# osudrl/cassie-mujoco-sim

Measured on AMD Instinct MI355X. Metric: env-steps/sec (whole node) at N envs; max |qpos_err| vs CPU ref, higher is better.
Workload: dtype f64

## Files before the change

### cassie-mujoco-sim_amd/csrc/env_step_rows.inc

```
        int r_ = lane;
        int rtype = -1, rid = 0, rsub = 0;
        int nefc = 0, nefc_before_contacts = 0;
        double rpos = 0, rmargin = 0, rR = 1.0, rK = 0, rB = 0, rimp = 1.0;
        const bool need_imu = lastsub || io.all_outputs_every_substep || (io.drive_mode && sub + 2 == nsub);
        const bool need_pos = lastsub || io.drive_mode || io.all_outputs_every_substep;
        const bool issens = lane < m->nsensor && need_pos;
        const int ls = issens ? lane : 0;
        SensorConsts sens_c;
        double ycol[NVP];
        double jvel = 0, jws = 0;
        const bool lastcol = !WIDE && lane == NROW - 1;
        for (int pass = 0; pass < (WIDE ? 2 : 1); ++pass) {
        if constexpr (WIDE) {
            if (pass == 1 && nefc <= NROW) break;
            r_ = NROW * pass + lane; rtype = -1; rid = 0; rsub = 0; nefc = 0; jvel = 0; jws = 0;
            rpos = 0; rmargin = 0; rR = 1.0; rK = 0; rB = 0; rimp = 1.0;
        }
        {
            const int neq = m->neq;
            const bool eact = lane < neq && m->eq_active[lane < neq ? lane : 0] != 0;
            const unsigned long long eall = neq >= 64 ? ~0ull : (1ull << neq) - 1;
            if (wv::ballot(eact) == eall && 3 * neq <= capr) {
                if (r_ < 3 * neq) { rtype = CM_CNSTR_EQUALITY; rid = r_ / 3; rsub = r_ - 3 * rid; }
                nefc = 3 * neq;
            } else
            for (int e = 0; e < neq; ++e) {
                if (!m->eq_active[e]) continue;
                if (nefc + 3 > capr) { warn |= WARN_CONSTRAINT_FULL; continue; }
                if (r_ >= nefc && r_ < nefc + 3) { rtype = CM_CNSTR_EQUALITY; rid = e; rsub = r_ - nefc; }
                nefc += 3;
            }
        }
        {
            for (unsigned long long any = lob | hib; any; any &= any - 1) {
                const int j = wv::popc64((any & (0ull - any)) - 1);
                for (int side = 0; side < 2; ++side) {
                    if (!(((side == 0 ? lob : hib) >> j) & 1ull)) continue;
                    if (nefc >= capr) { warn |= WARN_CONSTRAINT_FULL; continue; }
                    if (r_ == nefc) { rtype = CM_CNSTR_LIMIT_JOINT; rid = j; rsub = side; }
                    ++nefc;
                }
            }
        }
        nefc_before_contacts = nefc;
        const bool cpyr = lane < ncon && S.c_dim[lane < ncon ? lane : 0] == 3;
        if (wv::ballot(cpyr) == (ncon >= 64 ? ~0ull : (1ull << ncon) - 1) && nefc + 4 * ncon <= capr) {
            if (r_ >= nefc && r_ < nefc + 4 * ncon) { rtype = CM_CNSTR_CONTACT_PYRAMIDAL; rid = (r_ - nefc) >> 2; rsub = (r_ - nefc) & 3; }
            nefc += 4 * ncon;
        } else
        for (int c = 0; c < ncon; ++c) {
            const int dim = S.c_dim[c];
            if (dim != 1 && dim != 3) { warn |= WARN_UNSUPPORTED_PAIR; continue; }
            const int nrow = dim == 1 ? 1 : 2 * (dim - 1);
            if (nefc + nrow > capr) { warn |= WARN_CONSTRAINT_FULL; continue; }
            if (r_ >= nefc && r_ < nefc + nrow) {
                rtype = dim == 1 ? CM_CNSTR_CONTACT_FRICTIONLESS : CM_CNSTR_CONTACT_PYRAMIDAL;
                rid = c; rsub = r_ - nefc;
            }
            nefc += nrow;
        }

        CK_STAMP(25);
        double u3[3] = {0, 0, 0}, wp[3] = {0, 0, 0}, wm[3] = {0, 0, 0};
        unsigned long long maskp = 0, maskm = 0;
        int limdof = -1;
        double limsgn = 0, rdiag = 0, imp_pos = 0, rRscale = 1.0;
        double solref0 = 0.02, solref1 = 1, solimp[5] = {0.9, 0.95, 0.001, 0.5, 2};
        if (rtype == CM_CNSTR_EQUALITY) {
            if (rid != pf_eq) {
                pf_eb1 = m->eq_body1[rid]; pf_eb2 = m->eq_body2[rid]; pf_er1 = m->eq_root[rid][0]; pf_er2 = m->eq_root[rid][1];
            }
            maskp = m->eq_dofmask[rid][0]; maskm = m->eq_dofmask[rid][1];
            rdiag = P->eq_invweight[rid];
            solref0 = m->eq_solref[rid][0]; solref1 = m->eq_solref[rid][1];
            for (int i = 0; i < 5; ++i) solimp[i] = m->eq_solimp[rid][i];
            const int b1 = pf_eb1, b2 = pf_eb2;
            double l1[3] = {m->eq_data[rid][0], m->eq_data[rid][1], m->eq_data[rid][2]};
            double l2[3] = {m->eq_data[rid][3], m->eq_data[rid][4], m->eq_data[rid][5]};
            double a1[3], a2[3];
            mulmatvec3(a1, S.x.s.xmat[b1], l1);
            mulmatvec3(a2, S.x.s.xmat[b2], l2);
            for (int i = 0; i < 3; ++i) { a1[i] += S.x.s.xpos[b1][i]; a2[i] += S.x.s.xpos[b2][i]; }
            u3[0] = rsub == 0 ? 1.0 : 0.0; u3[1] = rsub == 1 ? 1.0 : 0.0; u3[2] = rsub == 2 ? 1.0 : 0.0;
            const double *c1 = S.com[pf_er1], *c2 = S.com[pf_er2];
            double o1[3] = {a1[0] - c1[0], a1[1] - c1[1], a1[2] - c1[2]};
            double o2[3] = {a2[0] - c2[0], a2[1] - c2[1], a2[2] - c2[2]};
            cross3(wp, o1, u3);
            cross3(wm, o2, u3);

            double res[3] = {a1[0] - a2[0], a1[1] - a2[1], a1[2] - a2[2]};
            rpos = rsub == 0 ? res[0] : (rsub == 1 ? res[1] : res[2]); rmargin = 0;
            imp_pos = sqrt(dot3(res, res));

        } else if (rtype == CM_CNSTR_LIMIT_JOINT) {
            const double q = S.qpos[m->jnt_qposadr[rid]];
            rpos = rsub == 0 ? q - m->jnt_range[rid][0] : m->jnt_range[rid][1] - q;
            rmargin = m->jnt_margin[rid];
            imp_pos = rpos;
            limdof = m->jnt_dofadr[rid];
            limsgn = rsub == 0 ? 1.0 : -1.0;
            rdiag = P->jnt_liminvweight[rid];
            solref0 = m->jnt_solref[rid][0]; solref1 = m->jnt_solref[rid][1];
            for (int i = 0; i < 5; ++i) solimp[i] = m->jnt_solimp[rid][i];
        } else if (rtype >= 0) {
            const int c = rid;
            const double *fr = S.c_frame[c];
            if (rtype == CM_CNSTR_CONTACT_PYRAMIDAL) {
                const int a = 1 + rsub / 2;
                const double mu = a <= 2 ? S.c_fri[c][0] : (a == 3 ? S.c_fri[c][1] : S.c_fri[c][2]);
                const double sg = (rsub & 1) ? -mu : mu;
                for (int i = 0; i < 3; ++i) u3[i] = fr[i] + sg * fr[3 * a + i];
                const double mu0 = S.c_fri[c][0];
                rRscale = 2 * mu0 * mu0;
            } else {
                for (int i = 0; i < 3; ++i) u3[i] = fr[i];
            }
            const double *c1 = S.com[S.c_root[c][0]], *c2 = S.com[S.c_root[c][1]];
            double o1[3] = {S.c_pos[c][0] - c1[0], S.c_pos[c][1] - c1[1], S.c_pos[c][2] - c1[2]};
            double o2[3] = {S.c_pos[c][0] - c2[0], S.c_pos[c][1] - c2[1], S.c_pos[c][2] - c2[2]};
            cross3(wp, o2, u3);
            cross3(wm, o1, u3);
            maskp = S.c_dofmask[c][1];
            maskm = S.c_dofmask[c][0];
            rpos = S.c_dist[c]; rmargin = S.c_margin[c]; imp_pos = rpos;
            const double tran = S.c_tran[c];
            const double mu_first = S.c_fri[c][0];
            rdiag = rtype == CM_CNSTR_CONTACT_PYRAMIDAL ? tran + mu_first * mu_first * tran : tran;
            solref0 = S.c_solref[c][0]; solref1 = S.c_solref[c][1];
            for (int i = 0; i < 5; ++i) solimp[i] = S.c_solimp[c][i];
        }
        CK_STAMP(26);
        if (rtype >= 0) {
            rimp = impedance(solimp, imp_pos, rmargin);
            rR = fmax(CM_MINVAL, (1 - rimp) * rdiag / rimp);
            if (rtype == CM_CNSTR_CONTACT_PYRAMIDAL) rR = fmax(CM_MINVAL, rRscale * rR);
            const double dmax = solimp[1];
            if (solref0 > 0) {
                double tc = solref0;
                if ((m->flags & CM_FLAG_REFSAFE) && tc < 2 * h) tc = 2 * h;
                rK = 1.0 / fmax(CM_MINVAL, dmax * dmax * tc * tc * solref1 * solref1);
                rB = 2.0 / fmax(CM_MINVAL, dmax * tc);
            } else {
                rK = -solref0 / fmax(CM_MINVAL, dmax * dmax);
                rB = -solref1 / fmax(CM_MINVAL, dmax);
            }
        }
        CK_STAMP(27);
        if constexpr (NW == 1) sens_c = request_sensor_consts(m, ls);
#pragma unroll
        for (int k0 = 0; k0 < NVP; k0 += 4) {
            double cc[4][6], qv[4], qw[4], qs[4];
#pragma unroll
            for (int kk = 0; kk < 4; ++kk) {
#pragma unroll
                for (int t = 0; t < 6; ++t) cc[kk][t] = S.cdof[k0 + kk][t];
                qv[kk] = S.qvel[k0 + kk]; qw[kk] = S.qacc_ws[k0 + kk];
                if constexpr (NW == 1) qs[kk] = S.qfrc_smooth[k0 + kk]; else qs[kk] = 0.0;
            }
            wv::sched_fence();
#pragma unroll
            for (int kk = 0; kk < 4; ++kk) {
                const int k = k0 + kk;
                double v = 0;
                if (TOPO::is_static ? k < TOPO::nv : k < nv) {
                    if (rtype >= 0) {
                        const double ul = u3[0] * cc[kk][3] + u3[1] * cc[kk][4] + u3[2] * cc[kk][5];
                        const double sp = bitf(maskp, k), sm = bitf(maskm, k);
                        v = sp * (ul + wp[0] * cc[kk][0] + wp[1] * cc[kk][1] + wp[2] * cc[kk][2]) -
                            sm * (ul + wm[0] * cc[kk][0] + wm[1] * cc[kk][1] + wm[2] * cc[kk][2]);
                        if (k == limdof) v = limsgn;
                        jvel += v * qv[kk];
                        jws += v * qw[kk];
                    } else if (lastcol) {
                        v = qs[kk];
                    }
                }
                ycol[k] = v;
            }
        }
        if constexpr (WIDE) {
            if (r_ < MAXR) {
#pragma unroll
                for (int k = 0; k < NVP; ++k) S.x.Yr[r_][k] = ycol[k];
                double *rt = S.x.rowt[r_];
                rt[0] = rR; rt[1] = rtype >= 0 ? -rB * jvel - rK * rimp * (rpos - rmargin) : 0.0; rt[2] = jws;
                rt[3] = rtype < 0 ? -1.0 : (rtype == CM_CNSTR_EQUALITY ? 0.0 : 1.0);
            }
            if (readout_ext<FEAT>(io) && pass == 0 && rtype == CM_CNSTR_EQUALITY && r_ < CM_MAXEQROW) {
                cm_ext_t *ex = readout_ext<FEAT>(io) + env;
                ex->eq_pos[r_] = rpos; ex->eq_id[r_] = rid;
#pragma unroll
                for (int k = 0; k < NVP; ++k) if (k < nv) ex->eq_J[r_][k] = ycol[k];
            }
        }
        }
        const int sb = NW == 1 ? sens_c.sb : 0;
        CK_STAMP(28);
        if constexpr (NW == 2) {
            if constexpr (WIDE) { if (lane == 0) S.x.turn[0] = nefc; }
            CK_STAMP(34); wv::block_barrier();
            if (lastcol) {
#pragma unroll
                for (int k = 0; k < NVP; ++k) ycol[k] = (TOPO::is_static ? k < TOPO::nv : k < nv) ? S.qfrc_smooth[k] : 0.0;
            }
        }
        const double raref = rtype >= 0 ? -rB * jvel - rK * rimp * (rpos - rmargin) : 0.0;

        int aslot = -1;
        if constexpr (NW == 1) aslot = sensors_before_solve(io, S, m, env, issens, ls, sens_c, need_imu, lastsub);
        CK_STAMP(29);
        if (io.xpos_out && isbody && lastsub) {
            for (int i = 0; i < 3; ++i) io.xpos_out[((size_t)env * io.sb + b) * 3 + i] = S.x.s.xpos[b][i];
            if (io.xquat_out) for (int i = 0; i < 4; ++i) io.xquat_out[((size_t)env * io.sb + b) * 4 + i] = S.x.s.xquat[b][i];
        }
        if (readout_ext<FEAT>(io)) {
            cm_ext_t *ex = readout_ext<FEAT>(io) + env;
            if (isbody) for (int i = 0; i < 6; ++i) ex->cvel[b][i] = S.x.s.cvel[b][i];
            if (isbody) for (int i = 0; i < 3; ++i) { ex->subtree_com[b][i] = S.com[broot > 0 ? broot : 0][i]; ex->xipos[b][i] = S.x.s.xipos[b][i]; }
            if (lane < m->nsite) {
                const int sb = m->site_bodyid[lane];
                double sp[3] = {m->site_pos[lane][0], m->site_pos[lane][1], m->site_pos[lane][2]};
                double sq[4] = {m->site_quat[lane][0], m->site_quat[lane][1], m->site_quat[lane][2], m->site_quat[lane][3]};
                double t[3], q[4], mm[9];
                mulmatvec3(t, S.x.s.xmat[sb], sp);
                for (int i = 0; i < 3; ++i) ex->site_xpos[lane][i] = t[i] + S.x.s.xpos[sb][i];
                mulquat(q, S.x.s.xquat[sb], sq);
                quat2mat(mm, q);
                for (int i = 0; i < 9; ++i) ex->site_xmat[lane][i] = mm[i];
            }
            if (isdof) for (int i = 0; i < 6; ++i) { ex->cdof[k_][i] = S.cdof[k_][i]; ex->cdof_dot[k_][i] = S.x.s.cdof_dot[k_][i]; }
            if (!WIDE && rtype == CM_CNSTR_EQUALITY && r_ < CM_MAXEQROW) {
                ex->eq_pos[r_] = rpos; ex->eq_id[r_] = rid;
#pragma unroll
                for (int k = 0; k < NVP; ++k) if (k < nv) ex->eq_J[r_][k] = ycol[k];
            }
            if (lane == 0) { int ne = 0; for (int e = 0; e < m->neq; ++e) if (m->eq_active[e] && ne + 3 <= capr) ne += 3; ex->ne = ne; }
            if (lane < ncon) {
                ex->con_geom1[lane] = m->geom_fullid[S.c_g1[lane]]; ex->con_geom2[lane] = m->geom_fullid[S.c_g2[lane]];
                ex->con_body1[lane] = m->geom_bodyid[S.c_g1[lane]]; ex->con_body2[lane] = m->geom_bodyid[S.c_g2[lane]];
                ex->con_dim[lane] = S.c_dim[lane]; ex->con_dist[lane] = S.c_dist[lane];
                for (int i = 0; i < 3; ++i) ex->con_pos[lane][i] = S.c_pos[lane][i];
                for (int i = 0; i < 9; ++i) ex->con_frame[lane][i] = S.c_frame[lane][i];
            }
        }
        int caddr = -1;
        const bool want_cfrc = io.body_cfrc && (sub == nsub - 1 || !integrates<FEAT>(io));
        if (readout_ext<FEAT>(io) || want_cfrc || sums) {
            int acc = nefc_before_contacts;
            for (int c = 0; c < ncon; ++c) {
                const int dim = S.c_dim[c];
                if (dim != 1 && dim != 3) continue;
                const int nrow = dim == 1 ? 1 : 2 * (dim - 1);
                if (acc + nrow > capr) continue;
                if (c == lane) caddr = acc;
                acc += nrow;
            }
        }
        wv::sync();
        CK_STAMP(8);
```

### cassie-mujoco-sim_amd/csrc/physics_kernel.h

```cpp
#ifndef CASSIE_PHYSICS_KERNEL_H
#define CASSIE_PHYSICS_KERNEL_H

#include <wave.h>

#include "cm_model.h"
#include "topo_static.h"

#include "pk_types.h"
#include "pk_math.h"
#include "pk_safety.h"
#include "pk_collision.h"
#include "pk_factor_solve.h"
#include "pk_stages.h"
#include "pk_wide_solve.h"

namespace ck {


constexpr int ENV_STEP_WENT_DOWN = 1 << 20;

template <int NVP, class TOPO, int FEAT, int MAXR, int NW>
WV_DEVICE int env_step(const PhysIO &io, EnvShared<NVP, LPack<TOPO, NVP>::count, MAXR> &S, int env, int sub_start, int nsub) {
    typedef LPack<TOPO, NVP> LP;
    static_assert(NW == 1 || NW == 2, "one or two wavefronts per env");
    static_assert(NW == 1 || TOPO::is_static, "the two-wave form exists for the compile-time topologies");
    const int wid = NW == 2 ? wv::wave_id() : 0;
    if constexpr (NW == 2) { if (wid == 0) wv::set_priority<CK_PRIO_W0>(); }
    constexpr int prio_kin = (FEAT & FEAT_HFIELD) != 0 ? CK_PRIO_W0 : CK_PRIO_W0_KIN;

    static_assert(LP::covers() && LP::distinct(), "packed factor rows must hold every ancestor pair, each in its own slot");
    typedef EnvShared<NVP, LPack<TOPO, NVP>::count, MAXR> SH_T;
    constexpr int MAXC = SH_T::MAXC;
    constexpr bool WIDE = SH_T::WIDE;
    static_assert(!WIDE || (NW == 2 && MAXR == WIDE_ROWS), "the 127-row instantiation spreads its solve over the two wavefronts of an env");
    constexpr bool sensors_behind_j = NW == 2 && !WIDE && (NVP <= 32 || CK_SENSORS_BEHIND_J_40DOF != 0) &&
                                      ((FEAT & FEAT_HFIELD) == 0 || CK_SENSORS_BEHIND_J_HFIELD != 0);
    const ModelPtr m_launch = (ModelPtr)(io.models + (size_t)env * io.model_stride);
    ModelPtr m = m_launch;
    const ParamPtr P = io.envparams ? (ParamPtr)(io.envparams + (size_t)env) : (ParamPtr)&m_launch->params;
    const ParamPtr PG = m_launch->env_geom ? P : (ParamPtr)&m_launch->params, PS = m_launch->env_springs ? P : (ParamPtr)&m_launch->params;
    int lane = wv::lane();
    const int nq = m->nq, nv = m->nv, nu = m->nu, nbody = m->nbody, njnt = m->njnt;
    const int capr = m->maxefc < MAXR ? m->maxefc : MAXR, capc = m->maxcon < MAXC ? m->maxcon : MAXC;
    const bool can_hand_over = MAXR < WIDE_ROWS && io.has_next != 0 && io.progress != nullptr && (MAXR < m->maxefc || MAXC < m->maxcon);
    const double h = m->timestep;
    int warn = 0;

    if (NW == 1 || wid == 0) {
    if (lane == 0) { S.cmd[0] = 0; S.cmd[1] = 0; S.cmd[2] = 0; S.cmd[3] = 0; S.cmd[4] = 0; }
    if constexpr (sensors_behind_j) { if (lane == 0) S.cmd[6] = 0; }
    if constexpr (WIDE) { if (lane == 0) { S.x.turn[0] = 0; S.x.turn[1] = 0; S.x.turn[2] = 0; S.x.turn[3] = 0; } }
    if (lane < nq) S.qpos[lane] = io.qpos[(size_t)env * io.sq + lane];
    if (lane < nv) {
        S.qvel[lane] = io.qvel[(size_t)env * io.sqv + lane];
        S.qacc_ws[lane] = io.qacc_warmstart[(size_t)env * io.sv + lane];
    }
    if (lane < nu) S.ctrl[lane] = io.ctrl[(size_t)env * io.su + lane];
    if (lane < NB && !wv::test_skip_com_init()) { S.com[lane][0] = 0.0; S.com[lane][1] = 0.0; S.com[lane][2] = 0.0; }
    if (io.drive_mode) {
        if (lane < m->nsensordata) S.sens[lane] = io.sensordata[(size_t)env * io.ssd + lane];
        if (lane < nu) S.actvel[lane] = io.actuator_velocity[(size_t)env * io.su + lane];
        drive_state_load(io, S, env, lane);
        drive_consts_load(io, S, m, env, lane);
    }
    }
    double time = io.time[env];

    int b = lane;
    bool isbody = b < nbody;
    const int depth = isbody ? m->body_depth[b] : -1;
    const int bparent = isbody ? m->body_parentid[b] : 0;
    const int broot = isbody ? m->body_rootid[b] : -1;
    const int bjn = isbody ? m->body_jntnum[b] : 0;
    const int bj0 = (isbody && bjn > 0) ? m->body_jntadr[b] : 0;
    const int bend = isbody ? m->body_subtreeend[b] : 0;
    const unsigned long long bdofmask = isbody ? m->body_dofmask[b] : 0ull;
    const int bjt = (isbody && bjn > 0) ? m->jnt_type[bj0] : -1;
    const int bjq = (isbody && bjn > 0) ? m->jnt_qposadr[bj0] : 0;
    int k_ = lane;
    bool isdof = k_ < nv;
    const int kjnt = isdof ? m->dof_jntid[k_] : 0;
    const int kbody = isdof ? m->dof_bodyid[k_] : 0;
    const int kjt = isdof ? m->jnt_type[kjnt] : -1;
    const int kda = isdof ? m->jnt_dofadr[kjnt] : 0;
    const int kqa = isdof ? m->jnt_qposadr[kjnt] : 0;
    const int kroot = isdof ? m->body_rootid[kbody] : 0;
    const int kbend = isdof ? m->body_subtreeend[kbody] : 0;
    const unsigned long long kdesc = isdof ? m->dof_descmask[k_] : 0ull;
    const unsigned long long kvelmask = isdof ? m->dof_velmask[k_] : 0ull;
    int kact = -1;
    for (int u = 0; u < nu; ++u) if (isdof && m->act_dofid[u] == k_) kact = u;
    const LaneIds ids = {nbody, nv, broot, bend, kjnt, kbody, kjt, kda, kroot, kbend, kdesc};
    wv::sync();

#include "env_step_wave1.inc"

    const float *env_hfield = nullptr;
    if constexpr ((FEAT & FEAT_HFIELD) != 0) {
        bool clamped;
        env_hfield = terrain_grid(io.hfield, io.hfield_stride, io.hfield_index, io.hfield_nterrain, env, &clamped);
        if (clamped && lane == 0 && wid == 0) wv::atomic_or(io.warn + env, WARN_TERRAIN_INDEX);
    }

    double *const sums = sums_row<FEAT>(io, env);

    bool bailed = false, bailed_down = false;
    int sub = sub_start;
    for (; sub < nsub; ++sub) {
        const bool lastsub = sub == nsub - 1 || !integrates<FEAT>(io);
        const bool need_quat = lastsub || readout_ext<FEAT>(io) != nullptr || io.all_outputs_every_substep || (io.drive_mode && sub + 2 == nsub);
        {
            bool badv = false;
            if (lane < nq) { double v = S.qpos[lane]; badv |= !(v == v) || fabs(v) > 1e10; }
            if (lane < nv) { double v = S.qvel[lane]; badv |= !(v == v) || fabs(v) > 1e10; }
            if (wv::ballot(badv) != 0ull) {
                warn |= WARN_DIVERGED;
                if constexpr (NW == 2) { if (lane == 0) S.cmd[0] = 1; wv::block_barrier(); }
                break;
            }
// ... 235 lines not shown
                for (int k = 1; k < NVP; ++k) {
                    if (TOPO::is_static ? k >= TOPO::nv : k >= nv) continue;
                    if (k > k_) { S.Lp[CK_TRI(k, k_)] = col[k]; S.LHp[CK_TRI(k, k_)] = colh[k]; }
                }
            }
        }
        if constexpr (NW == 1) CK_STAMP(4);

#include "env_step_collision.inc"

        double mycvel[6], mycacc[6];
#pragma unroll
        for (int r = 0; r < 3 * chain_rounds; ++r) { wv::keep(danc[r]); if (!isdof) danc[r] = -1; }
        wv::keep(blast); wv::keep(kvin);
        if (!isbody) blast = -1;
        if (!isdof) kvin = -1;
        const int kd = isdof ? k_ : 0;
        const double kdamp = P->dof_damping[kd], kstiff = PS->dof_stiffness[kd], kref = PS->dof_springref[kd];
        const double kgear = m->dof_gear[kd], klo = m->dof_ctrl_lo[kd], khi = m->dof_ctrl_hi[kd];
        const int kq = m->dof_qadr[kd], ka = m->dof_act[kd];
        auto chain_sums = [&](double (&acc)[6]) {
            if (lane < NVP) for (int t = 0; t < 6; ++t) S.x.s.buf[lane][t] = acc[t];
            wv::sync();
#pragma unroll
            for (int r = 0; r < chain_rounds; ++r) {
                double up[3][6];
#pragma unroll
                for (int i = 0; i < 3; ++i) {
                    const int a = danc[3 * r + i] >= 0 ? danc[3 * r + i] : 0;
                    for (int t = 0; t < 6; ++t) up[i][t] = S.x.s.buf[a][t];
                }
                wv::sync();
#pragma unroll
                for (int i = 0; i < 3; ++i)
                    if (danc[3 * r + i] >= 0) for (int t = 0; t < 6; ++t) acc[t] += up[i][t];
                if (lane < NVP) for (int t = 0; t < 6; ++t) S.x.s.buf[lane][t] = acc[t];
                wv::sync();
            }
        };
        {
            double term[6];
            const double qd = isdof ? S.qvel[lane < NVP ? lane : 0] : 0.0;
            for (int t = 0; t < 6; ++t) term[t] = (lane < NVP ? S.cdof[lane < NVP ? lane : 0][t] : 0.0) * qd;
            chain_sums(term);
            for (int t = 0; t < 6; ++t) mycvel[t] = blast >= 0 ? S.x.s.buf[blast >= 0 ? blast : 0][t] : 0.0;
            double vin[6];
            for (int t = 0; t < 6; ++t) vin[t] = kvin >= 0 ? S.x.s.buf[kvin >= 0 ? kvin : 0][t] : 0.0;
            if (lane < NB) for (int t = 0; t < 6; ++t) S.x.s.cvel[lane][t] = mycvel[t];
            if (lane < NVP) {
                double cdd[6] = {0, 0, 0, 0, 0, 0}, cd[6];
                for (int i = 0; i < 6; ++i) cd[i] = S.cdof[lane][i];
                if (isdof && !(kjt == CM_JNT_FREE && k_ - kda < 3)) cross_motion(cdd, vin, cd);
                for (int i = 0; i < 6; ++i) S.x.s.cdof_dot[lane][i] = cdd[i];
                for (int t = 0; t < 6; ++t) term[t] = cdd[t] * qd;
            } else {
                for (int t = 0; t < 6; ++t) term[t] = 0;
            }
            wv::sync();
            CK_STAMP(23);
            chain_sums(term);
            for (int t = 0; t < 6; ++t) mycacc[t] = blast >= 0 ? S.x.s.buf[blast >= 0 ? blast : 0][t] : 0.0;
            mycacc[3] -= m->gravity[0]; mycacc[4] -= m->gravity[1]; mycacc[5] -= m->gravity[2];
            wv::sync();
            if (lane < NB) for (int t = 0; t < 6; ++t) S.x.s.buf[lane][t] = mycacc[t];
            wv::sync();
        }
        if (lane < NB) {
            double f6[6] = {0, 0, 0, 0, 0, 0};
            if (isbody && b > 0) {
                double t1[6], t2[6], t3[6], ci[10];
                for (int i = 0; i < 10; ++i) ci[i] = S.x.s.cinert[b][i];
                mul_inert_vec(t1, ci, mycacc);
                mul_inert_vec(t2, ci, mycvel);
                cross_force(t3, mycvel, t2);
                for (int i = 0; i < 6; ++i) f6[i] = t1[i] + t3[i];
            }
            for (int i = 0; i < 6; ++i) S.x.s.cfrc[lane][i] = f6[i];
        }
        wv::sync();
        CK_STAMP(24);
        if constexpr (NW == 2) {
            wv::publish(&S.cmd[1], sub + 1);
        } else bias_forces_and_qfrc_smooth<NVP, FEAT>(io, S, m, env, ids, kdamp, kstiff, kref, kgear, klo, khi, kq, ka);
        const int pf_eq = lane < 3 * m->neq ? lane / 3 : 0;
        int pf_eb1 = m->eq_body1[pf_eq], pf_eb2 = m->eq_body2[pf_eq], pf_er1 = m->eq_root[pf_eq][0], pf_er2 = m->eq_root[pf_eq][1];

#include "env_step_rows.inc"

#include "env_step_solve.inc"

    if constexpr (feat_sums(FEAT)) { if (sums && lane == 0 && sub > sub_start) sums[CM_SUM_COUNT] = sums[CM_SUM_COUNT] + (double)(sub - sub_start); }
    if (io.progress && lane == 0 && (!io.resume || bailed)) {
        io.progress[env] = bailed ? sub : nsub;
        if (bailed && !bailed_down && io.handover_out_list) io.handover_out_list[io.env0 + wv::atomic_add(io.handover_out_count, 1)] = env;
    }
    if (integrates<FEAT>(io) && io.drive_mode) {
        drive_state_store(io, S, env, lane);
        if (lane < nu) io.ctrl[(size_t)env * io.su + lane] = S.ctrl[lane];
        if (bailed) {
            if (lane < m->nsensordata) io.sensordata[(size_t)env * io.ssd + lane] = S.sens[lane];
            if (lane < nu) io.actuator_velocity[(size_t)env * io.su + lane] = S.actvel[lane];
            if (lane < CM_NUM_DRIVES) {
                double *meas = io.meas + (size_t)env * CM_MEAS_DIM;
                meas[CM_MEAS_DRIVE_POS + lane] = S.drv_pos[lane]; meas[CM_MEAS_DRIVE_VEL + lane] = S.drv_vel[lane];
            }
        }
    }
    if (integrates<FEAT>(io)) {
        if (lane < nq) io.qpos[(size_t)env * io.sq + lane] = S.qpos[lane];
        if (lane < nv) {
            io.qvel[(size_t)env * io.sqv + lane] = S.qvel[lane];
            io.qacc_warmstart[(size_t)env * io.sv + lane] = S.qacc_ws[lane];
        }
        if (lane == 0) io.time[env] = time;
    }
    {
        int w = 0;
        for (int bit = 1; bit <= 8; bit <<= 1)
            if (wv::ballot((warn & bit) != 0) != 0ull) w |= bit;
        if (lane == 0 && w) io.warn[env] |= w;
    }
    return (warn & WARN_DIVERGED) ? -2 : (bailed ? (bailed_down ? sub | ENV_STEP_WENT_DOWN : sub) : nsub);
}

template <int NVP, class TOPO, int FEAT = FEAT_ALL, int MAXR = MID_ROWS, int NW = 1, bool WALK = false, int WPS = NW, int INROWS = 0, int SERVE = FEAT_FULL>
WV_GLOBAL void __launch_bounds__(WV_WAVE * NW) WV_OCC WV_WAVES_PER_SIMD(WPS) cassie_step_kernel(PhysIO io) {
    static_assert((FEAT & FEAT_SERVE) == 0 && (SERVE & ~FEAT_SERVE) == 0, "FEAT: the collision bits; SERVE: FEAT_READOUT / FEAT_PROF / FEAT_SUMS");
    WV_SHARED EnvShared<NVP, LPack<TOPO, NVP>::count, MAXR> S;
    const int slot = wv::env_id();
    if constexpr (WALK) {
        wv::test_launch_hook(&S, sizeof S);
        const int count = wv::opaque(wv::shfl_i(wv::lane() == 0 ? wv::atomic_add(io.handover_count, 0) : 0, 0));
        for (int idx = slot; idx < count; idx += wv::grid_size()) {
            const int env = io.handover_list[io.env0 + idx];
            const long long t0 = io.cost ? wv::clock() : 0, t0w = io.cost_wall ? wv::wall_clock() : 0;
            env_step<NVP, TOPO, FEAT | SERVE, MAXR, NW>(io, S, env, io.progress[env], io.nsub);
            if (io.cost && wv::lane() == 0 && (NW == 1 || wv::wave_id() == 0)) {
                io.cost[env] += (unsigned)((wv::clock() - t0) >> 6);
                if (io.cost_wall) io.cost_wall[env] += (unsigned)(wv::wall_clock() - t0w);
            }
            if constexpr (NW == 2) wv::block_barrier();
            else wv::sync();
        }
        if (wv::lane() == 0 && (NW == 1 || wv::wave_id() == 0) && wv::atomic_add(io.handover_count + 1, 1) == wv::grid_size() - 1) {
            io.handover_count[0] = 0; io.handover_count[1] = 0;
            if (io.handover_seen) *io.handover_seen = count;
        }
    } else {
    const int chunk = io.nchunk > 1 ? wv::env_id() / io.nenv : 0;
    const int eslot = slot - chunk * io.nenv;
    if (chunk >= (io.nchunk > 1 ? io.nchunk : 1)) return;
    wv::test_launch_hook(&S, sizeof S);
    const int env = io.order ? io.order[io.env0 + eslot] : io.env0 + eslot;
    int sub_start = io.resume ? io.progress[env] : 0, sub_end = io.nsub;
    if (io.nchunk > 1) {
        const int per = (io.nsub + io.nchunk - 1) / io.nchunk;
        sub_start = chunk * per;
        sub_end = sub_start + per < io.nsub ? sub_start + per : io.nsub;
    }
    if (sub_start >= io.nsub) return;
    if (chunk > 0) {
        if (!wv::wait_global<NW>(io.chunk_flag + env, io.chunk_seq, chunk)) {
            if (wv::lane() == 0) { wv::atomic_or(io.warn + env, WARN_CHUNK_PLACEMENT); if (io.chunk_fault) *io.chunk_fault = 1; }
        }
        if (io.progress[env] != sub_start) {
            if (sub_end < io.nsub) wv::publish_global<NW>(io.chunk_flag + env, io.chunk_seq, chunk + 1);
            return;
// ... 50 lines not shown
```

### cassie-mujoco-sim_amd/csrc/pk_types.h

```cpp
#ifndef CASSIE_PK_TYPES_H
#define CASSIE_PK_TYPES_H

#ifndef WV_HAS_WAIT_FOR_STRAIGHT
namespace wv { inline void wait_for_straight(const int *flag, int value) { wait_for(flag, value); } }
#endif

namespace ck {

constexpr int NB = CM_MAXBODY;
constexpr int NG = CM_MAXGEOM;
constexpr int NROW = 64;
constexpr int MID_ROWS = CM_MAXEFC_NARROW;
constexpr int WIDE_ROWS = CM_MAXEFC;
constexpr int FAST_ROWS = 31;
constexpr int FAST_ROWS_TRAY = 47;
constexpr int NSTAMP = 48;
#ifndef CK_SENSORS_BEHIND_J_40DOF
#define CK_SENSORS_BEHIND_J_40DOF 0
#endif
#ifndef CK_SENSORS_BEHIND_J_HFIELD
#define CK_SENSORS_BEHIND_J_HFIELD 0
#endif
#define CK_TRI(k, i) ((k) * ((k) + 1) / 2 + (i))
#define CK_STAMP(i) do { if constexpr (feat_prof(FEAT)) { if (io.prof && lane == 0) io.prof[(size_t)env * NSTAMP + (i)] = wv::clock(); } CK_FRESH(); } while (0)
#define CK_FRESH() do { lane = wv::fresh_lane(); b = lane; k_ = lane; isbody = b < nbody; isdof = k_ < nv; } while (0)

enum { WARN_CONTACT_FULL = 1, WARN_CONSTRAINT_FULL = 2, WARN_UNSUPPORTED_PAIR = 4, WARN_DIVERGED = 8,
       WARN_CHUNK_PLACEMENT = 16 ,
       WARN_TERRAIN_INDEX = 32   ,
       WARN_SCAN_TILTED = 64     ,
       WARN_PLACE_MISS = 128      };

#ifndef WV_OCC
#define WV_OCC
#endif
typedef const WV_CONST_AS cm_model_t *ModelPtr;
typedef const WV_CONST_AS cm_envparams_t *ParamPtr;

struct PhysIO {
    const cm_model_t *models;
    int model_stride;
    const cm_envparams_t *envparams;
    int nenv, nsub;
    int env0;
    int integrate;
    int sq, sqv, sv, su, ssd, sb;
    double *qpos, *qvel, *qacc_warmstart, *time;
    double *ctrl;
    const double *qfrc_applied, *xfrc_applied;
    double *qacc, *sensordata, *actuator_velocity;
    int *warn;
    int *info;
    double *xpos_out;
    double *xquat_out;
    double *body_cfrc;
    const float *hfield;
    size_t hfield_stride;
    const double *pd_ptarget, *pd_kp, *pd_kd;
    int drive_mode;
    cm_drive_state_t *drive_state;
    const double *drive_cmd;
    const double *pd_dtarget, *pd_torque;
    double *meas;
    cm_ext_t *ext;
    long long *prof;
    const int *order;
    unsigned *cost;
    unsigned *cost_wall;
    int all_outputs_every_substep;
    int *progress;
    int resume;
    int nchunk, chunk_seq;
    int *chunk_flag;
    volatile int *chunk_fault;
    int *handover_list, *handover_count;
    volatile int *handover_seen;
    int has_next;
    int *handover_out_list, *handover_out_count;
    int inplace_has_next;
    int *inplace_out_list, *inplace_out_count;
    int inplace_stay_rows;
    int down_rows;
    int *inplace_count;
    const int *hfield_index;
    int hfield_nterrain;
    double *sums;
    int sums_stride;
};

WV_DEVICE const float *terrain_grid(const float *hfield, size_t stride, const int *index, int nterrain, int env, bool *clamped) {
    *clamped = false;
    if (!hfield) return nullptr;
    if (!index) return hfield + (size_t)env * stride;
    const int want = index[env], last = nterrain - 1;
    const int t = want > last ? last : (want < 0 ? 0 : want);
    *clamped = t != want;
    return hfield + (size_t)(t < 0 ? 0 : t) * stride;
}

template <int NVP>
struct BodyTiles {
    double xpos[NB][3], xquat[NB][4], xmat[NB][9], xipos[NB][3];
    double xanchor[CM_MAXJNT][3], xaxis[CM_MAXJNT][3];
    double cinert[NB][10], crb[NB][10];
    double cvel[NB][6], cfrc[NB][6];
    double cdof_dot[NVP][6], buf[NVP][6];
// ... 49 lines not shown
```

### cassie-mujoco-sim_amd/csrc/wave.h

```cpp
#ifndef CASSIE_WAVE_H
#define CASSIE_WAVE_H

#include <hip/hip_runtime.h>

#define WV_DEVICE __device__ __forceinline__
#define WV_GLOBAL __global__
#define WV_SHARED __shared__
#define WV_WAVE 64
#define WV_WAVES_PER_SIMD(n) __attribute__((amdgpu_waves_per_eu(n)))
#define WV_CONST_AS __attribute__((address_space(4)))

namespace wv {

WV_DEVICE int lane() { return (int)(threadIdx.x & 63u); }
WV_DEVICE int wave_id() { return __builtin_amdgcn_readfirstlane((int)(threadIdx.x >> 6)); }
WV_DEVICE void publish(int *flag, int value) {
    __builtin_amdgcn_fence(__ATOMIC_RELEASE, "workgroup", "local");
    if (threadIdx.x % 64u == 0) *(volatile int *)flag = value;
}
WV_DEVICE void wait_for(const int *flag, int value) {
    while (__builtin_amdgcn_readfirstlane(*(const volatile int *)flag) != value) __builtin_amdgcn_s_sleep(1);
    __builtin_amdgcn_fence(__ATOMIC_ACQUIRE, "workgroup", "local");
}
#define WV_HAS_WAIT_FOR_STRAIGHT 1
// ... 44 lines not shown
        }
    }
    if (NW > 1) __builtin_amdgcn_s_barrier();
    __builtin_amdgcn_fence(__ATOMIC_ACQUIRE, "agent");
    __builtin_amdgcn_s_dcache_inv();
#ifdef CK_CHUNK_RELEASE_AGENT
    return true;
#else
    return threadIdx.x >= 64u || ((word >> 3) & 7) == xcc_id();
#endif
}
WV_DEVICE int fresh_lane() {
    int x;
    asm volatile("v_mbcnt_lo_u32_b32 %0, -1, 0\n\tv_mbcnt_hi_u32_b32 %0, -1, %0" : "=v"(x));
    return x;
}
#ifndef CK_PRIO
#define CK_PRIO 1
#endif
#ifndef CK_PRIO_W0
#define CK_PRIO_W0 1
#endif
#ifndef CK_PRIO_W0_KIN
#define CK_PRIO_W0_KIN 3
#endif
#ifndef CK_PRIO_W0_PGS
#define CK_PRIO_W0_PGS CK_PRIO_W0
#endif
#ifndef CK_PRIO_W1_FJ
#define CK_PRIO_W1_FJ 1
#endif
#ifndef CK_PRIO_W1_FJ_HFIELD
#define CK_PRIO_W1_FJ_HFIELD 0
#endif
#ifndef CK_PRIO_W1_JP
#define CK_PRIO_W1_JP 0
#endif
#ifndef CK_PRIO_W1_PE
#define CK_PRIO_W1_PE 3
#endif
#ifndef CK_PRIO_W1_EF
#define CK_PRIO_W1_EF 0
#endif
template <int P> WV_DEVICE void set_priority() { if (CK_PRIO) __builtin_amdgcn_s_setprio(P); }
WV_DEVICE int env_id() { return (int)blockIdx.x; }
WV_DEVICE int grid_size() { return (int)gridDim.x; }
WV_DEVICE int atomic_add(int *p, int v) { return atomicAdd(p, v); }
WV_DEVICE int atomic_or(int *p, int v) { return atomicOr(p, v); }

WV_DEVICE void sync() {
    __builtin_amdgcn_fence(__ATOMIC_RELEASE, "wavefront");
    __builtin_amdgcn_wave_barrier();
    __builtin_amdgcn_fence(__ATOMIC_ACQUIRE, "wavefront");
}

WV_DEVICE double shfl(double v, int src_lane) { return __shfl(v, src_lane, WV_WAVE); }
WV_DEVICE double shfl_xor(double v, int mask) { return __shfl_xor(v, mask, WV_WAVE); }
WV_DEVICE int shfl_i(int v, int src_lane) { return __shfl(v, src_lane, WV_WAVE); }

struct mfma_acc { double c[4]; };
WV_DEVICE void mfma_f64_16x16x4(double a, double b, mfma_acc &c) {
    typedef double d4 __attribute__((ext_vector_type(4)));
    d4 x = {c.c[0], c.c[1], c.c[2], c.c[3]};
    x = __builtin_amdgcn_mfma_f64_16x16x4f64(a, b, x, 0, 0, 0);
    c.c[0] = x[0]; c.c[1] = x[1]; c.c[2] = x[2]; c.c[3] = x[3];
}
WV_DEVICE void mfma_f64_16x16x4_x3(double a0, double b0, mfma_acc &c0, double a1, double b1, mfma_acc &c1, double a2, double b2, mfma_acc &c2) {
    mfma_f64_16x16x4(a0, b0, c0); mfma_f64_16x16x4(a1, b1, c1); mfma_f64_16x16x4(a2, b2, c2);
}
WV_DEVICE void mfma_f64_16x16x4_x4(double a0, double b0, mfma_acc &c0, double a1, double b1, mfma_acc &c1, double a2, double b2, mfma_acc &c2,
                                   double a3, double b3, mfma_acc &c3) {
    mfma_f64_16x16x4(a0, b0, c0); mfma_f64_16x16x4(a1, b1, c1); mfma_f64_16x16x4(a2, b2, c2); mfma_f64_16x16x4(a3, b3, c3);
}
WV_DEVICE void mfma_f64_drain(mfma_acc &, mfma_acc &, mfma_acc &) {}
WV_DEVICE void mfma_f64_drain4(mfma_acc &, mfma_acc &, mfma_acc &, mfma_acc &) {}

WV_DEVICE double from_upper_half(double v) {
    const int lo = __double2loint(v), hi = __double2hiint(v);
    const auto rl = __builtin_amdgcn_permlane32_swap(lo, lo, false, false);
    const auto rh = __builtin_amdgcn_permlane32_swap(hi, hi, false, false);
    return __hiloint2double((int)rh[1], (int)rl[1]);
}

WV_DEVICE double readlane(double v, int src) {
    int lo = __double2loint(v), hi = __double2hiint(v);
    lo = __builtin_amdgcn_readlane(lo, src);
    hi = __builtin_amdgcn_readlane(hi, src);
    return __hiloint2double(hi, lo);
}

template <int DST> WV_DEVICE double writelane(double v, double s) {
    int lo = __double2loint(v), hi = __double2hiint(v);
    const int slo = __builtin_amdgcn_readfirstlane(__double2loint(s)), shi = __builtin_amdgcn_readfirstlane(__double2hiint(s));
    asm("v_writelane_b32 %0, %1, %2" : "+v"(lo) : "s"(slo), "n"(DST));
    asm("v_writelane_b32 %0, %1, %2" : "+v"(hi) : "s"(shi), "n"(DST));
    return __hiloint2double(hi, lo);
}

template <int CTRL, int ROW_MASK> WV_DEVICE float dpp_take_f32(float v) {
    return __int_as_float(__builtin_amdgcn_update_dpp(0, __float_as_int(v), CTRL, ROW_MASK, 0xf, false));
}
WV_DEVICE float wave_sum_f32(float v) {
    v += dpp_take_f32<0xB1, 0xf>(v);
    v += dpp_take_f32<0x4E, 0xf>(v);
    v += dpp_take_f32<0x141, 0xf>(v);
    v += dpp_take_f32<0x140, 0xf>(v);
    v += dpp_take_f32<0x142, 0xa>(v);
    v += dpp_take_f32<0x143, 0xc>(v);
    return __int_as_float(__builtin_amdgcn_readlane(__float_as_int(v), 63));
}

WV_DEVICE unsigned long long ballot(bool p) { return __ballot(p); }

template <int CTRL, int ROW_MASK> WV_DEVICE double dpp_take(double v) {
    const int lo = __builtin_amdgcn_update_dpp(0, __double2loint(v), CTRL, ROW_MASK, 0xf, false);
    const int hi = __builtin_amdgcn_update_dpp(0, __double2hiint(v), CTRL, ROW_MASK, 0xf, false);
    return __hiloint2double(hi, lo);
}

WV_DEVICE double wave_sum(double v) {
    v += dpp_take<0xB1, 0xf>(v);
    v += dpp_take<0x4E, 0xf>(v);
    v += dpp_take<0x141, 0xf>(v);
    v += dpp_take<0x140, 0xf>(v);
    v += dpp_take<0x142, 0xa>(v);
    v += dpp_take<0x143, 0xc>(v);
    return readlane(v, 63);
}

WV_DEVICE double mul_rn(double a, double b) { return __dmul_rn(a, b); }
WV_DEVICE double add_rn(double a, double b) { return __dadd_rn(a, b); }
WV_DEVICE double sub_rn(double a, double b) { return __dsub_rn(a, b); }
WV_DEVICE double div_rn(double a, double b) { return __ddiv_rn(a, b); }
WV_DEVICE double sqrt_rn(double a) { return __dsqrt_rn(a); }

WV_DEVICE double rcp_estimate(double x) { return __builtin_amdgcn_rcp(x); }
WV_DEVICE double rsq_estimate(double x) { return __builtin_amdgcn_rsq(x); }

WV_DEVICE int opaque(int x) { x = __builtin_amdgcn_readfirstlane(x); asm volatile("" : "+s"(x)); return x; }

template <class P> WV_DEVICE P opaque_ptr(P p) {
    const unsigned long long v = (unsigned long long)p;
    unsigned lo = __builtin_amdgcn_readfirstlane((unsigned)v), hi = __builtin_amdgcn_readfirstlane((unsigned)(v >> 32));
    asm volatile("" : "+s"(lo), "+s"(hi));
    return (P)(((unsigned long long)hi << 32) | lo);
}

WV_DEVICE void keep(int &x) { asm volatile("" : "+v"(x)); }

WV_DEVICE void touch(double x) { asm volatile("" : : "v"(x)); }

WV_DEVICE void sched_fence() { __builtin_amdgcn_sched_barrier(0); }

WV_DEVICE constexpr bool debug_force_guarded() { return false; }
WV_DEVICE constexpr bool test_skip_com_init() { return false; }
template <class S> WV_DEVICE void test_launch_hook(S *, unsigned long) {}

WV_DEVICE long long clock() { return (long long)__builtin_readcyclecounter(); }
WV_DEVICE long long wall_clock() { return (long long)__builtin_readsteadycounter(); }
WV_DEVICE long long hw_id() {
    unsigned hw, xcc;
    asm volatile("s_getreg_b32 %0, hwreg(HW_REG_HW_ID)" : "=s"(hw));
    asm volatile("s_getreg_b32 %0, hwreg(HW_REG_XCC_ID)" : "=s"(xcc));
    return (long long)(((unsigned long long)xcc << 32) | hw);
}

WV_DEVICE int popc64(unsigned long long x) { return __popcll(x); }
WV_DEVICE double max_raw(double a, double b) { double r; asm("v_max_f64 %0, %1, %2" : "=v"(r) : "v"(a), "v"(b)); return r; }

}
#endif
```

Measured before the change: 28.36 million.

## Split constraint Jacobian row build across wave halves, each computing half the DOFs

When there are at most 31 constraint rows and 32 static DOFs, both 32-lane halves of the wavefront compute the same row. Each half covers 16 of the DOF columns, and the halves swap results with permlane32_swap. Motion-axis data is read with 16-byte paired LDS loads. The aim is to halve the per-lane Jacobian column loop and the cdof LDS traffic, since upper lanes would otherwise hold empty rows. In exchange it adds cross-half swaps, extra bookkeeping to reset the upper-half row state, and a serial dot-product tail over the swapped half.

New measurement: 28.61 million, median of 6. No clear change (+0.9%).

```diff
diff --git a/cassie-mujoco-sim_amd/csrc/env_step_rows.inc b/cassie-mujoco-sim_amd/csrc/env_step_rows.inc
--- a/cassie-mujoco-sim_amd/csrc/env_step_rows.inc
+++ b/cassie-mujoco-sim_amd/csrc/env_step_rows.inc
@@ -16,6 +16,7 @@
             r_ = NROW * pass + lane; rtype = -1; rid = 0; rsub = 0; nefc = 0; jvel = 0; jws = 0;
             rpos = 0; rmargin = 0; rR = 1.0; rK = 0; rB = 0; rimp = 1.0;
         }
+        if constexpr (jrows_halves) r_ = lane & 31;
         {
             const int neq = m->neq;
             const bool eact = lane < neq && m->eq_active[lane < neq ? lane : 0] != 0;
@@ -147,6 +148,59 @@
         }
         CK_STAMP(27);
         if constexpr (NW == 1) sens_c = request_sensor_consts(m, ls);
+        if constexpr (jrows_halves) {
+            constexpr int NH = NVP / 2;
+            const int kofs = lane >= NROW / 2 ? NH : 0;
+            const unsigned mp16 = (unsigned)(maskp >> kofs), mm16 = (unsigned)(maskm >> kofs);
+            const int limk = limdof - kofs;
+            static_assert(offsetof(SH_T, cdof) % 16 == 0 && alignof(SH_T) <= 16, "the motion axes start on a 16-byte boundary of the env's LDS block");
+            int cpair = 3 * kofs;
+            wv::keep(cpair);
+            const double *const cdh = &S.cdof[0][0] + 2 * cpair;
+            double vh[NH];
+#pragma unroll
+            for (int i = 0; i < NH; ++i) vh[i] = 0;
+            if (rtype >= 0) {
+#pragma unroll
+                for (int i0 = 0; i0 < NH; i0 += 4) {
+                    double cc[4][6], qv[4], qw[4];
+#pragma unroll
+                    for (int kk = 0; kk < 4; ++kk) {
+#pragma unroll
+                        for (int t = 0; t < 6; t += 2) wv::load_pair16(cdh + 6 * (i0 + kk) + t, cc[kk][t], cc[kk][t + 1]);
+                        qv[kk] = S.qvel[i0 + kk]; qw[kk] = S.qacc_ws[i0 + kk];
+                    }
+                    wv::sched_fence();
+#pragma unroll
+                    for (int kk = 0; kk < 4; ++kk) {
+                        const int i = i0 + kk;
+                        const double ul = u3[0] * cc[kk][3] + u3[1] * cc[kk][4] + u3[2] * cc[kk][5];
+                        const double sp = (double)((mp16 >> i) & 1u), sm = (double)((mm16 >> i) & 1u);
+                        double v = sp * (ul + wp[0] * cc[kk][0] + wp[1] * cc[kk][1] + wp[2] * cc[kk][2]) -
+                                   sm * (ul + wm[0] * cc[kk][0] + wm[1] * cc[kk][1] + wm[2] * cc[kk][2]);
+                        if (i == limk) v = limsgn;
+                        jvel += v * qv[kk];
+                        jws += v * qw[kk];
+                        vh[i] = v;
+                    }
+                }
+            }
+#pragma unroll
+            for (int i = 0; i < NH; ++i) wv::pair_halves(vh[i], ycol[i], ycol[NH + i]);
+#pragma unroll
+            for (int k = NH; k < NVP; ++k) { jvel += ycol[k] * S.qvel[k]; jws += ycol[k] * S.qacc_ws[k]; }
+            if constexpr (NW == 1) {
+                if (lastcol) {
+#pragma unroll
+                    for (int k = 0; k < NVP; ++k) ycol[k] = S.qfrc_smooth[k];
+                }
+            }
+            r_ = lane;
+            if (lane >= NROW / 2) {
+                rtype = -1; rid = 0; rsub = 0; jvel = 0; jws = 0;
+                rpos = 0; rmargin = 0; rR = 1.0; rK = 0; rB = 0; rimp = 1.0;
+            }
+        } else {
 #pragma unroll
         for (int k0 = 0; k0 < NVP; k0 += 4) {
             double cc[4][6], qv[4], qw[4], qs[4];
@@ -178,6 +232,7 @@
                 ycol[k] = v;
             }
         }
+        }
         if constexpr (WIDE) {
             if (r_ < MAXR) {
 #pragma unroll
diff --git a/cassie-mujoco-sim_amd/csrc/physics_kernel.h b/cassie-mujoco-sim_amd/csrc/physics_kernel.h
--- a/cassie-mujoco-sim_amd/csrc/physics_kernel.h
+++ b/cassie-mujoco-sim_amd/csrc/physics_kernel.h
@@ -35,6 +35,8 @@
     static_assert(!WIDE || (NW == 2 && MAXR == WIDE_ROWS), "the 127-row instantiation spreads its solve over the two wavefronts of an env");
     constexpr bool sensors_behind_j = NW == 2 && !WIDE && (NVP <= 32 || CK_SENSORS_BEHIND_J_40DOF != 0) &&
                                       ((FEAT & FEAT_HFIELD) == 0 || CK_SENSORS_BEHIND_J_HFIELD != 0);
+    constexpr bool jrows_halves = CK_JROWS_HALVES != 0 && MAXR <= 31 && NVP == 32 && !WIDE && TOPO::is_static && TOPO::nv == NVP &&
+                                  ((FEAT & FEAT_HFIELD) == 0 || CK_JROWS_HALVES_HFIELD != 0);
     const ModelPtr m_launch = (ModelPtr)(io.models + (size_t)env * io.model_stride);
     ModelPtr m = m_launch;
     const ParamPtr P = io.envparams ? (ParamPtr)(io.envparams + (size_t)env) : (ParamPtr)&m_launch->params;
@@ -436,7 +438,8 @@
         if constexpr (NW == 2) {
             wv::publish(&S.cmd[1], sub + 1);
         } else bias_forces_and_qfrc_smooth<NVP, FEAT>(io, S, m, env, ids, kdamp, kstiff, kref, kgear, klo, khi, kq, ka);
-        const int pf_eq = lane < 3 * m->neq ? lane / 3 : 0;
+        int pf_eq = lane < 3 * m->neq ? lane / 3 : 0;
+        if constexpr (jrows_halves) pf_eq = (lane & 31) < 3 * m->neq ? (lane & 31) / 3 : 0;
         int pf_eb1 = m->eq_body1[pf_eq], pf_eb2 = m->eq_body2[pf_eq], pf_er1 = m->eq_root[pf_eq][0], pf_er2 = m->eq_root[pf_eq][1];
 
 #include "env_step_rows.inc"
diff --git a/cassie-mujoco-sim_amd/csrc/pk_types.h b/cassie-mujoco-sim_amd/csrc/pk_types.h
--- a/cassie-mujoco-sim_amd/csrc/pk_types.h
+++ b/cassie-mujoco-sim_amd/csrc/pk_types.h
@@ -3,6 +3,12 @@
 
 #ifndef WV_HAS_WAIT_FOR_STRAIGHT
 namespace wv { inline void wait_for_straight(const int *flag, int value) { wait_for(flag, value); } }
+#endif
+#ifndef WV_HAS_LOAD_PAIR16
+namespace wv { inline void load_pair16(const double *p, double &a, double &b) { a = p[0]; b = p[1]; } }
+#endif
+#ifndef WV_HAS_PAIR_HALVES
+namespace wv { inline void pair_halves(double v, double &lo, double &hi) { const double o = shfl_xor(v, 32); const bool low = lane() < 32; lo = low ? v : o; hi = low ? o : v; } }
 #endif
 
 namespace ck {
@@ -21,7 +27,13 @@
 #ifndef CK_SENSORS_BEHIND_J_HFIELD
 #define CK_SENSORS_BEHIND_J_HFIELD 0
 #endif
-#define CK_TRI(k, i) ((k) * ((k) + 1) / 2 + (i))
+#ifndef CK_JROWS_HALVES
+#define CK_JROWS_HALVES 1
+#endif
+#ifndef CK_JROWS_HALVES_HFIELD
+#define CK_JROWS_HALVES_HFIELD 0
+#endif
+#define CK_TRI(k, i)((k) * ((k) + 1) / 2 + (i))
 #define CK_STAMP(i) do { if constexpr (feat_prof(FEAT)) { if (io.prof && lane == 0) io.prof[(size_t)env * NSTAMP + (i)] = wv::clock(); } CK_FRESH(); } while (0)
 #define CK_FRESH() do { lane = wv::fresh_lane(); b = lane; k_ = lane; isbody = b < nbody; isdof = k_ < nv; } while (0)
 
diff --git a/cassie-mujoco-sim_amd/csrc/wave.h b/cassie-mujoco-sim_amd/csrc/wave.h
--- a/cassie-mujoco-sim_amd/csrc/wave.h
+++ b/cassie-mujoco-sim_amd/csrc/wave.h
@@ -150,6 +150,15 @@
     return __hiloint2double((int)rh[1], (int)rl[1]);
 }
 
+#define WV_HAS_PAIR_HALVES 1
+WV_DEVICE void pair_halves(double v, double &lo, double &hi) {
+    const int l = __double2loint(v), h = __double2hiint(v);
+    const auto rl = __builtin_amdgcn_permlane32_swap(l, l, false, false);
+    const auto rh = __builtin_amdgcn_permlane32_swap(h, h, false, false);
+    lo = __hiloint2double((int)rh[0], (int)rl[0]);
+    hi = __hiloint2double((int)rh[1], (int)rl[1]);
+}
+
 WV_DEVICE double readlane(double v, int src) {
     int lo = __double2loint(v), hi = __double2hiint(v);
     lo = __builtin_amdgcn_readlane(lo, src);
@@ -218,6 +227,13 @@
 
 WV_DEVICE void touch(double x) { asm volatile("" : : "v"(x)); }
 
+#define WV_HAS_LOAD_PAIR16 1
+WV_DEVICE void load_pair16(const double *p, double &a, double &b) {
+    typedef double d2 __attribute__((ext_vector_type(2)));
+    const d2 v = *(const d2 *)__builtin_assume_aligned(p, 16);
+    a = v[0]; b = v[1];
+}
+
 WV_DEVICE void sched_fence() { __builtin_amdgcn_sched_barrier(0); }
 
 WV_DEVICE constexpr bool debug_force_guarded() { return false; }
```
